# keras-team/keras-rs

Hardware: AMD Instinct MI355X
Metric: embedding lookups/sec + DCN fwd+bwd step time, 26-table DLRM batch 65 536 (higher is better)
Workload: dtype bf16; 1 GPU; C3 DLRM-small: 26 tables x 1000000 rows x 128 (bf16), global batch 65536, multi-hot ml_perf lengths (sum L = 214), uniform ids, DotInteraction(F=27) + 3 x FeatureCross(d=3456, projection=512), fused Adagrad on tables; global_batch=65536, parallelism=single GPU

## Files before the change

### include/krs.h

```cpp
#ifndef KRS_H_
#define KRS_H_

#include <stddef.h>
#include <stdint.h>

#ifdef __cplusplus
extern "C" {
#endif

#define KRS_VERSION 100

typedef enum krs_status {
  KRS_OK = 0,
  KRS_ERR_INVALID = -1,
  KRS_ERR_UNSUPPORTED = -2,
  KRS_ERR_LAUNCH = -3,
  KRS_ERR_WORKSPACE = -4
} krs_status;

typedef enum krs_dtype { KRS_F32 = 0, KRS_BF16 = 1, KRS_I8 = 2 } krs_dtype;
typedef enum krs_itype { KRS_I32 = 0, KRS_I64 = 1 } krs_itype;

typedef enum krs_combiner { KRS_SUM = 0, KRS_MEAN = 1, KRS_SQRTN = 2 } krs_combiner;

// ... 178 lines not shown

enum {
  KRS_GEMM_KERNEL_NONE = 0, KRS_GEMM_KERNEL_GENERIC = 1, KRS_GEMM_KERNEL_MFMA = 2, KRS_GEMM_KERNEL_GLDS = 3,
  KRS_GEMM_KERNEL_TN_GLDS = 4, KRS_GEMM_KERNEL_PP256 = 5, KRS_GEMM_KERNEL_PP256_KSTRIDED = 6, KRS_GEMM_KERNEL_PP64 = 7,
  KRS_GEMM_KERNEL_THIN = 8, KRS_GEMM_KERNEL_ROWDOT = 9, KRS_GEMM_KERNEL_SMALLK = 10
};
enum { KRS_GEMM_REDUCE_NONE = 0, KRS_GEMM_REDUCE_SCALAR = 1, KRS_GEMM_REDUCE_VEC4 = 2, KRS_GEMM_REDUCE_VEC8 = 3 };
typedef struct krs_gemm_route {
  int32_t kernel;
  int32_t splits;
  int32_t reduce;
  int32_t epilogue;
  int32_t ep_vec;
  int32_t thin_width;
  int32_t thin_is_a;
} krs_gemm_route;
int krs_gemm_last_route(krs_gemm_route* route);
int krs_gemm_plan_route(const void* a, int64_t lda, int a_is_km, const void* b, int64_t ldb, int b_is_nk, const void* c,
                        int64_t ldc, int64_t m, int64_t n, int64_t k, int in_dtype, int out_dtype,
                        const krs_gemm_epilogue* epilogue, size_t workspace_bytes, krs_gemm_route* route);

enum { KRS_GEMM_OPT_PIPELINE = 0 };
int krs_gemm_set_option(int key, int value);

enum { KRS_EMBED_OPT_PLAN = 2, KRS_EMBED_OPT_HOTROWS = 3, KRS_EMBED_OPT_RANK = 4, KRS_EMBED_OPT_APPLY_DEPTH = 5 };
int krs_embed_set_option(int key, int value);

size_t krs_colsum_workspace_bytes(int64_t m, int64_t n);
int krs_cross_epilogue_fwd(const void* u, const void* x0, const void* x, void* y,
                           int64_t m, int64_t n, int64_t ld, float diag_scale,
                           int dtype, void* stream);
int krs_cross_epilogue_bwd(const void* g, const void* u, const void* x0, const void* x,
                           void* du, void* dx0, int dx0_accumulate, void* dxd,
                           float* dbias,
                           int64_t m, int64_t n, int64_t ld, float diag_scale, int act,
                           int dtype, void* workspace, size_t workspace_bytes, void* stream);

// ... 215 lines not shown
```

### keras_rs_amd/_lib.py

```python

from __future__ import annotations

import ctypes as C
import os

import numpy as np
import torch

_HERE = os.path.dirname(os.path.abspath(__file__))
LIB_PATH = os.environ.get("KRS_LIB", os.path.join(_HERE, "libkrs_hip.so"))

F32, BF16, I8 = 0, 1, 2
I32, I64 = 0, 1
SUM, MEAN, SQRTN = 0, 1, 2
COMBINERS = {"sum": SUM, "mean": MEAN, "sqrtn": SQRTN}
ACT_NONE, ACT_RELU, ACT_SIGMOID, ACT_TANH = 0, 1, 2, 3
FLAG_ID_OUT_OF_RANGE = 1
FLAG_BAD_OFFSETS = 2
FLAG_CAPACITY_OVERFLOW = 4
FLAG_NONFINITE_ROW = 8
MAX_LIST = 4096

TABLE_DT = np.dtype(
    [("weights", "<u8"), ("slot", "<u8"), ("row_base", "<i8"), ("vocab", "<i4"), ("lr", "<f4")]
# ... 13 lines not shown
        ("act", C.c_int32),
        ("diag_scale", C.c_float),
        ("x0", C.c_void_p),
        ("x", C.c_void_p),
        ("ldx", C.c_int64),
        ("u_out", C.c_void_p),
        ("ldu", C.c_int64),
        ("r", C.c_void_p),
        ("ldr", C.c_int64),
        ("beta", C.c_float),
    ]


class GemmRoute(C.Structure):
    _fields_ = [(name, C.c_int32) for name in
                ("kernel", "splits", "reduce", "epilogue", "ep_vec", "thin_width", "thin_is_a")]


class GemmQ8Route(C.Structure):
    _fields_ = [(name, C.c_int32) for name in ("kernel", "ep_vec", "k_tail", "epilogue")]


class EmbedFwdRoute(C.Structure):
    _fields_ = [(name, C.c_int32) for name in
                ("kernel", "lpr", "has_w", "stream", "hot_rows", "bpg", "table_dtype", "out_dtype")] + [("blocks", C.c_int64)]


class DotRoute(C.Structure):
    _fields_ = [(name, C.c_int32) for name in
                ("kernel", "dtype", "ks", "fr", "self", "multi", "acc", "ng", "lps_log2", "spw", "launches",
                 "lds_bytes")] + [("blocks", C.c_int64)]
# ... 203 lines not shown
```

### keras_rs_amd/csrc/gemm.hip

```cpp
#include <algorithm>
#include <cstdlib>
#include <cstring>

#include "gemm_device.h"
#include "gemm_plan.h"
#include "gemm_ring64.h"

namespace krs {
namespace {

constexpr int BM = gplan::kTile, BN = gplan::kTile;
constexpr int ROW_BYTES = gplan::kRowBytes;
constexpr int TILE_BYTES = gplan::kTileBytes;

template <int ES>
__device__ __forceinline__ void load_kstrided(const char* base, int64_t ld, int64_t row0, int64_t k0,
                                              int64_t rows, int64_t kk, u32x4 (&r)[4]) {
  constexpr int RPB = 16 / ES;
  constexpr int NRB = BM / RPB;
  const int t = threadIdx.x;
  const int rb = t % NRB;
  const int kb = t / NRB;
  const int64_t row = row0 + rb * RPB;
#pragma unroll
// ... 24 lines not shown
      const int j = jj;
      const int w = j >> 1;
      uint32_t lo, hi;
      if (j & 1) {
        lo = (r[0][w] >> 16) | (r[1][w] & 0xffff0000u);
        hi = (r[2][w] >> 16) | (r[3][w] & 0xffff0000u);
      } else {
        lo = (r[0][w] & 0xffffu) | (r[1][w] << 16);
        hi = (r[2][w] & 0xffffu) | (r[3][w] << 16);
      }
      *reinterpret_cast<uint2*>(tile + lds_chunk_off<true>(rb * 8 + j, kb >> 1) + (kb & 1) * 8) = make_uint2(lo, hi);
    }
  }
}

template <int EPI, int NPFC>
__device__ __forceinline__ void gemm_epilogue_wave128_pre(const GemmParams& p, f32x16 (&acc)[2][2][2], float* stage,
                                                          int64_t wm0, int64_t wn0, int split, EpiOperands (&o)[4]) {
  static_assert(NPFC == 2 || NPFC == 4, "two or four chunks of operands are fetched ahead");
  epi_process<EPI>(p, acc[0][0], o[0], stage, wm0, wn0, split);
  if constexpr (NPFC == 2) epi_prefetch<EPI>(p, o[2], wm0 + 64, wn0);
  epi_process<EPI>(p, acc[0][1], o[1], stage, wm0 + 32, wn0, split);
  if constexpr (NPFC == 2) epi_prefetch<EPI>(p, o[3], wm0 + 96, wn0);
  epi_process<EPI>(p, acc[1][0], o[2], stage, wm0 + 64, wn0, split);
  epi_process<EPI>(p, acc[1][1], o[3], stage, wm0 + 96, wn0, split);
}

template <int EPI>
__device__ __forceinline__ void gemm_epilogue(const GemmParams& p, f32x16 (&acc)[2][2], char* smem, int64_t m0,
                                              int64_t n0, int split) {
  const int wave = threadIdx.x >> 6;
  gemm_epilogue_wave<EPI>(p, acc, reinterpret_cast<float*>(smem) + wave * (32 * 68), m0 + (wave >> 1) * 64,
                          n0 + (wave & 1) * 64, split);
}

template <int ES, bool A_KM, bool B_NK, int EPI>
__global__ __launch_bounds__(256, 3) void gemm_mfma_kernel(const GemmParams p) {
  extern __shared__ __attribute__((aligned(16))) char smem[];
  constexpr int BK = ROW_BYTES / ES;
  auto tile_a = [&](int) -> char* { return smem; };
// ... 397 lines not shown
}
template <int N>
__device__ __forceinline__ void pp_lgkm_wait(u32x4 (&fa)[4], u32x4 (&fb)[2]) {
  asm volatile("s_waitcnt lgkmcnt(%6)"
               : "+v"(fa[0]), "+v"(fa[1]), "+v"(fa[2]), "+v"(fa[3]), "+v"(fb[0]), "+v"(fb[1])
               : "n"(N));
}

struct RingMmaBf16 {
  f32x16 (&acc)[2][2][2];
  __device__ __forceinline__ void operator()(int i, int j, const u32x4& fa, const u32x4& fb) const {
    f32x16& d = acc[i >> 1][i & 1][j];
    d = __builtin_amdgcn_mfma_f32_32x32x16_bf16(__builtin_bit_cast(bf16x8, fa), __builtin_bit_cast(bf16x8, fb), d, 0, 0, 0);
  }
};
template <int EPI> constexpr int kRingEpiChunks = EPI == 2 ? 4 : EPI == 1 ? 2 : 0;
template <int EPI> constexpr int kRingEpiLoads = kRingEpiChunks<EPI> * (EPI == 1 ? 8 : 4);

template <bool TN, int NSTG, int EPI>
__global__ __launch_bounds__(512) void gemm_pp256_kernel(const GemmParams p, int mt, int nt) {
  extern __shared__ __attribute__((aligned(16))) char smem[];
  constexpr int TM = 256, TN_ = 256;
  typedef const __attribute__((address_space(1))) void* gptr;
  typedef __attribute__((address_space(3))) void* lptr;

  const int lane = threadIdx.x & 63;
  const int wave = __builtin_amdgcn_readfirstlane(threadIdx.x >> 6);
  const int grp = wave >> 2;
  const int wm = grp, wn = wave & 3;
  const int64_t xcd = blockIdx.x & 7, slot = blockIdx.x >> 3;
  int64_t m0, n0, kbeg = 0, nkb;
// ... 203 lines not shown
  }
  lds_dma_retired<NPF>();
  float* stage_f = reinterpret_cast<float*>(smem) + wave * (32 * 68);
  if constexpr (EPI >= 3) {
    gemm_epilogue_wave128_crossbwd<(EPI == 4 || EPI == 6) ? 1 : (EPI == 7 ? 2 : (EPI >= 8 ? 3 : 0)),
                                   EPI == 3 || EPI == 4 || EPI == 7, EPI < 9, EPI != 9>(
        p, acc, stage_f, m0 + wm * 128, n0 + wn * 64, (m0 >> 8) * 2 + wm);
    return;
  }
  if constexpr (NPFC > 0)
    gemm_epilogue_wave128_pre<EPI, NPFC>(p, acc, stage_f, m0 + wm * 128, n0 + wn * 64, split, opf);
  else
    gemm_epilogue_wave128<EPI>(p, acc, stage_f, m0 + wm * 128, n0 + wn * 64, split);
}

template <int EPI>
__global__ __launch_bounds__(512) void gemm_pp64_kernel(const GemmParams p, int nt) {
  extern __shared__ __attribute__((aligned(16))) char smem[];
  constexpr int TM = 256, TN_ = 256;
  const int lane = threadIdx.x & 63;
  const int wave = __builtin_amdgcn_readfirstlane(threadIdx.x >> 6);
  const int wm = wave >> 2, wn = wave & 3;
  const int64_t xcd = blockIdx.x & 7, slot_id = blockIdx.x >> 3;
  const int64_t tslot = slot_id / p.splits;
  const int split = (int)(slot_id - tslot * p.splits);
  const int64_t m_tile = (tslot / nt) * 8 + xcd;
  if (m_tile * TM >= p.m) return;
  const int64_t m0 = m_tile * TM, n0 = (tslot % nt) * TN_;
  const int64_t kbeg = (int64_t)split * p.k_per_split;
  const int64_t nb = (min(p.k, kbeg + p.k_per_split) - kbeg) / 64;

  f32x16 acc[2][2][2];
#pragma unroll
  for (int h = 0; h < 2; ++h)
#pragma unroll
    for (int i = 0; i < 2; ++i)
#pragma unroll
      for (int j = 0; j < 2; ++j)
#pragma unroll
        for (int r = 0; r < 16; ++r) acc[h][i][j][r] = 0.0f;
  constexpr int NPFC = kRingEpiChunks<EPI>;
  EpiOperands opf[4];
  ring64_main_loop<2, kRingEpiLoads<EPI>>(smem, p, m0, n0, kbeg, nb, lane, wave, RingMmaBf16{acc}, [&]() {
#pragma unroll
    for (int c = 0; c < NPFC; ++c) epi_prefetch<EPI>(p, opf[c], m0 + wm * 128 + c * 32, n0 + wn * 64);
  });
  float* stage_f = reinterpret_cast<float*>(smem) + wave * (32 * 68);
  if constexpr (EPI >= 3) {
    gemm_epilogue_wave128_crossbwd<(EPI == 4 || EPI == 6) ? 1 : (EPI == 7 ? 2 : (EPI >= 8 ? 3 : 0)),
                                   EPI == 3 || EPI == 4 || EPI == 7, EPI < 9, EPI != 9>(
        p, acc, stage_f, m0 + wm * 128, n0 + wn * 64, (m0 >> 8) * 2 + wm);
    return;
  }
  if constexpr (NPFC > 0)
    gemm_epilogue_wave128_pre<EPI, NPFC>(p, acc, stage_f, m0 + wm * 128, n0 + wn * 64, split, opf);
  else
    gemm_epilogue_wave128<EPI>(p, acc, stage_f, m0 + wm * 128, n0 + wn * 64, split);
}

template <int ES, int NT>
__global__ __launch_bounds__(256) void gemm_thin_kernel(const GemmParams p, int thin_is_a) {
  typedef typename std::conditional<ES == 2, uint16_t, float>::type elem_t;
  __shared__ __attribute__((aligned(16))) float thin[128][NT];
  const elem_t* wide_p = reinterpret_cast<const elem_t*>(thin_is_a ? p.b : p.a);
  const elem_t* thin_p = reinterpret_cast<const elem_t*>(thin_is_a ? p.a : p.b);
  const int64_t ldw = thin_is_a ? p.ldb : p.lda, ldt = thin_is_a ? p.lda : p.ldb;
  const int64_t n_wide = thin_is_a ? p.n : p.m;
  const int n_thin = (int)(thin_is_a ? p.m : p.n);
  const int64_t col = (int64_t)blockIdx.x * 256 + threadIdx.x;
  const int64_t ccol = col < n_wide ? col : n_wide - 1;
// ... 188 lines not shown
    const float bv = p.b_nk ? ld_elem(p.b, in_dtype, j * p.ldb + kk) : ld_elem(p.b, in_dtype, kk * p.ldb + j);
    acc = fmaf(av, bv, acc);
  }
  epilogue_store(p, i, j, acc);
}

int g_pipe = -1;
int gemm_pipe() {
  if (g_pipe < 0) {
    const char* e = getenv("KRS_GEMM_PIPE");
    g_pipe = e ? atoi(e) : 4;
    if (g_pipe != 0 && g_pipe != 5) g_pipe = 4;
  }
  return g_pipe;
}

template <int First, int Last, class F>
int with_epilogue(int e, F&& f) {
  if constexpr (First < Last) {
    if (e != First) return with_epilogue<First + 1, Last>(e, f);
  }
  return f(std::integral_constant<int, First>());
}

}
}

using namespace krs;

extern "C" int krs_gemm_set_option(int key, int value) {
  if (key == KRS_GEMM_OPT_PIPELINE) {
    KRS_REQUIRE(value == 0 || value == 4 || value == 5, "krs_gemm_set_option: pipeline must be 0, 4 or 5");
    g_pipe = value;
    return KRS_OK;
  }
  return fail(KRS_ERR_INVALID, "krs_gemm_set_option: unknown key %d", key);
}

extern "C" size_t krs_gemm_workspace_bytes(int64_t m, int64_t n, int64_t k, int a_is_km) {
  return gplan::plan_workspace_bytes(m, n, k, a_is_km != 0);
}

namespace krs {
namespace {
static_assert(gplan::kRingLds == 4 * pp::STAGE && gplan::kRing64Lds == ring64::NSLOT * ring64::SLOT, "the planner's LDS bytes");

thread_local krs_gemm_route g_route = {};

int gemm_plan(const void* a, int64_t lda, int a_is_km, const void* b, int64_t ldb, int b_is_nk, const void* c, int64_t ldc,
              int64_t m, int64_t n, int64_t k, int in_dtype, int out_dtype, const krs_gemm_epilogue* ep,
              size_t workspace_bytes, bool allow_split, gplan::GemmCall& call, gplan::GemmPlan& pl) {
  KRS_REQUIRE(a && b && c, "krs_gemm: null operand");
  KRS_REQUIRE(m >= 0 && n >= 0 && k >= 0, "krs_gemm: negative size");
  KRS_REQUIRE((in_dtype == KRS_F32 || in_dtype == KRS_BF16) && (out_dtype == KRS_F32 || out_dtype == KRS_BF16),
              "krs_gemm: bad dtype");
  if (ep && ep->x0) KRS_REQUIRE(ep->x, "krs_gemm: cross epilogue needs x with x0");
  static const bool tn128 = getenv("KRS_GEMM_TN128") != nullptr;
  call = gplan::GemmCall();
  call.m = m; call.n = n; call.k = k; call.a_km = a_is_km != 0; call.b_nk = b_is_nk != 0;
  call.es = in_dtype == KRS_BF16 ? 2 : 4; call.out_dtype = out_dtype;
  call.lda = lda; call.ldb = ldb; call.ldc = ldc; call.al_a = al16(a); call.al_b = al16(b); call.al_c = al16(c);
  gplan::set_epilogue(call, ep);
  call.workspace_bytes = workspace_bytes; call.allow_split = allow_split; call.pipe = gemm_pipe(); call.tn128 = tn128;
  pl = gplan::plan_gemm(call);
  if (pl.status == KRS_ERR_WORKSPACE)
    return fail(pl.status, "krs_gemm: split-K needs %zu workspace bytes, got %zu", pl.need, workspace_bytes);
  if (pl.status != KRS_OK) return fail(pl.status, "krs_gemm: the shape needs a grid beyond the launch limits");
  return KRS_OK;
}

template <int ES>
int gemm_launch(const GemmParams& p, const gplan::GemmPlan& pl, int in_dtype, hipStream_t st) {
  const krs_gemm_route& rt = pl.route;
  const dim3 grid((unsigned)pl.grid[0], (unsigned)pl.grid[1], (unsigned)pl.grid[2]), block((unsigned)pl.block);
  switch (rt.kernel) {
    case KRS_GEMM_KERNEL_PP64:
      return with_epilogue<0, 2>(rt.epilogue, [&](auto E) {
        return launch_lds<gemm_pp64_kernel<E>>("gemm_pp64_kernel", grid, block, pl.lds, st, p, pl.nt);
      });
    case KRS_GEMM_KERNEL_PP256:
      return with_epilogue<0, 2>(rt.epilogue, [&](auto E) {
        return launch_lds<gemm_pp256_kernel<false, 4, E>>("gemm_pp256_kernel", grid, block, pl.lds, st, p, 0, pl.nt);
      });
    case KRS_GEMM_KERNEL_PP256_KSTRIDED:
      return launch_lds<gemm_pp256_kernel<true, 4, 0>>("gemm_pp256_kernel (K-strided operands)", grid, block, pl.lds, st, p,
                                                       pl.mt, pl.nt);
    case KRS_GEMM_KERNEL_TN_GLDS:
      return launch_lds<gemm_tn_glds_kernel<0>>("gemm_tn_glds_kernel", grid, block, pl.lds, st, p, pl.mt, pl.nt);
    case KRS_GEMM_KERNEL_GLDS:
      return with_epilogue<0, 2>(rt.epilogue, [&](auto E) {
        return launch_lds<gemm_glds_kernel<ES, E>>("gemm_glds_kernel", grid, block, pl.lds, st, p);
      });
    case KRS_GEMM_KERNEL_MFMA:
      return with_epilogue<0, 2>(rt.epilogue, [&](auto E) {
// ... 97 lines not shown
                     gplan::CrossBwdPlan* plan_only = nullptr) {
  const bool store_g = g_out != nullptr;
  if (dense && !g_out) { g_out = dz; ldg = ld; }
  if (!r) { ldr = n; beta = 0.0f; }
  KRS_REQUIRE(dtype == KRS_BF16 || dtype == KRS_F32, "%s: bad dtype", who);
  KRS_REQUIRE(m >= 0 && n >= 0 && k > 0 && ld >= n && ldg >= n && ldr >= n, "%s: bad sizes", who);
  krs_gemm_epilogue ep;
  memset(&ep, 0, sizeof(ep));
  ep.r = r; ep.ldr = ldr; ep.beta = beta;
  gplan::CrossBwdPlan cb;
  if (m > 0 && n > 0) {
    gplan::GemmCall call;
    if (int rc = gemm_plan(a, lda, 0, bt, ldb, 1, g_out, ldg, m, n, k, dtype, dtype, r ? &ep : nullptr, 0, false, call, cb.product))
      return rc;
    gplan::plan_cross_bwd(cb, r != nullptr, ld, al16(x0) && al16(u) && al16(dz) && al16(dx0) && al16(u_upper), dense, store_g,
                          dx0 != nullptr, dx0_accumulate != 0, u_upper != nullptr);
  }
  if (plan_only) { *plan_only = cb; return KRS_OK; }
  if (dbias) KRS_REQUIRE(workspace_bytes >= krs_gemm_cross_bwd_workspace_bytes(m, n) && (workspace || m == 0 || n == 0),
                         "%s: workspace too small (krs_gemm_cross_bwd_workspace_bytes)", who);
  hipStream_t st = reinterpret_cast<hipStream_t>(stream);
  if (m == 0 || n == 0) {
    if (dbias && n > 0) KRS_HIP(hipMemsetAsync(dbias, 0, (size_t)n * sizeof(float), st));
    return KRS_OK;
  }
  if (cb.route == KRS_CROSS_BWD_TWO_CALL) {
    cb_route = cb.route;
    if (int rc = gemm_run(a, lda, 0, bt, ldb, 1, g_out, ldg, m, n, k, dtype, dtype, r ? &ep : nullptr, nullptr, 0, stream,
                          false))
      return rc;
    KRS_REQUIRE(ldg == ld, "%s: the two-call form needs one row stride for G, x0, u, dz and dx0", who);
// ... 4 lines not shown
      if (int rc = krs_cross_epilogue_bwd(r, u_upper, x0, x0, nullptr, dx0, 0, nullptr, nullptr, m, n, ld, 0.0f, KRS_ACT_NONE,
                                          dtype, nullptr, 0, stream)) return rc;
      dx0_accumulate = 1;
    }
    return krs_cross_epilogue_bwd(g_out, u, x0, x0, dz, dx0, dx0_accumulate, fold_direct ? dx0 : nullptr, dbias, m, n,
                                  ld, 0.0f, act, dtype, workspace, workspace_bytes, stream);
  }
  GemmParams p = gemm_params(a, lda, false, bt, ldb, true, g_out, ldg, m, n, k, KRS_BF16, &ep);
  p.ep_vec = 1;
  p.f_x0 = x0; p.f_u = u; p.f_uup = u_upper; p.f_dz = dz; p.f_dx0 = dx0; p.f_ld = ld; p.f_act = act; p.f_fold = fold_direct != 0;
  p.f_partial = dbias ? reinterpret_cast<float*>(workspace) : nullptr;
  const gplan::GemmPlan& pl = cb.product;
  const dim3 grid256((unsigned)pl.grid[0]), block((unsigned)pl.block);
  cb_route = cb.route; cb_epilogue = cb.epilogue;
  const int rc = with_epilogue<3, 10>(cb.epilogue, [&](auto E) {
    return cb.route == KRS_CROSS_BWD_PP64
               ? launch_lds<gemm_pp64_kernel<E>>("gemm_pp64_kernel (fused cross backward)", grid256, block, pl.lds, st, p, pl.nt)
               : launch_lds<gemm_pp256_kernel<false, 4, E>>("gemm_pp256_kernel (fused cross backward)", grid256, block, pl.lds,
                                                            st, p, 0, pl.nt);
  });
  if (rc != KRS_OK) return rc;
  return dbias ? finish_colsum(p.f_partial, 2 * ceil_div(m, 256), n, dbias, st) : KRS_OK;
}

extern "C" int krs_gemm_cross_bwd_plan_route(const void* a, int64_t lda, const void* bt, int64_t ldb, const void* r,
                                             int64_t ldr, float beta, void* g_out, int64_t ldg, const void* x0, const void* u,
                                             void* dz, void* dx0, int64_t ld, int dx0_accumulate, const void* u_upper,
                                             int64_t m, int64_t n, int64_t k, int dtype, int* epilogue) {
  gplan::CrossBwdPlan cb;
  const int rc = cross_bwd("krs_gemm_cross_bwd_plan_route", x0 == nullptr, a, lda, bt, ldb, r, ldr, beta, g_out, ldg, x0, u, dz,
                           dx0, ld, dx0_accumulate, u_upper, 0, nullptr, m, n, k, KRS_ACT_NONE, dtype, nullptr, 0, nullptr, &cb);
  if (epilogue) *epilogue = cb.epilogue;
  return rc ? rc : cb.route;
}
// ... 26 lines not shown
```

### keras_rs_amd/csrc/gemm_device.h

```cpp
#ifndef KRS_GEMM_DEVICE_H_
#define KRS_GEMM_DEVICE_H_

#include "gemm_plan.h"
#include "krs_dense_common.h"

namespace krs {
namespace {

typedef __bf16 bf16x8 __attribute__((ext_vector_type(8)));
typedef float f32x16 __attribute__((ext_vector_type(16)));
typedef uint32_t u32x4 __attribute__((ext_vector_type(4)));

struct GemmParams {
  const char* a; int64_t lda; int a_km;
  const char* b; int64_t ldb; int b_nk;
  char* c; int64_t ldc;
  int64_t m, n, k;
  int out_dtype;
  krs_gemm_epilogue ep;
  int has_ep;
  int splits; int64_t k_per_split; float* slabs;
  int ep_vec;
  const void* f_x0; const void* f_u; const void* f_uup; void* f_dz; void* f_dx0; float* f_partial; int64_t f_ld; int f_act; int f_fold;
};
// ... 120 lines not shown
    }
    if (e.r) {
      float rv[8];
      load8(e.r, odt, i * e.ldr + j, rv);
#pragma unroll
      for (int q = 0; q < 8; ++q) v[q] += e.beta * rv[q];
    }
  }
  store8(p.c, odt, i * p.ldc + j, v);
}


struct EpiOperands {
  uint4 ex[4], ex0[4];
};

template <int EPI>
__device__ __forceinline__ void epi_prefetch(const GemmParams& p, EpiOperands& o, int64_t row0, int64_t wn0) {
  if constexpr (EPI == 1 || EPI == 2) {
    const int lane = threadIdx.x & 63;
    const int64_t gnc = min(wn0 + (lane & 7) * 8, p.n - 8);
#pragma unroll
    for (int it = 0; it < 4; ++it) {
      const int64_t gmc = min(row0 + it * 8 + (lane >> 3), p.m - 1);
      if constexpr (EPI == 1) {
        o.ex[it] = load8_bf16_nt(p.ep.x, gmc * p.ep.ldx + gnc);
        o.ex0[it] = load8_bf16_nt(p.ep.x0, gmc * p.ep.ldx + gnc);
      } else {
        o.ex[it] = load8_bf16_nt(p.ep.r, gmc * p.ep.ldr + gnc);
      }
    }
  }
}

template <int EPI>
__device__ __forceinline__ void epi_process(const GemmParams& p, f32x16 (&acc2)[2], const EpiOperands& o, float* stage,
                                            int64_t row0, int64_t wn0, int split) {
  const int lane = threadIdx.x & 63;
  const int frow = lane & 31;
  const int fhalf = lane >> 5;
  constexpr int SST = 68;
  const int ec = (lane & 7) * 8;
  const int64_t gn = wn0 + ec;
#pragma unroll
  for (int j = 0; j < 2; ++j)
#pragma unroll
    for (int r = 0; r < 16; ++r)
      stage[((r & 3) + 8 * (r >> 2) + 4 * fhalf) * SST + j * 32 + frow] = acc2[j][r];
  __builtin_amdgcn_fence(__ATOMIC_ACQ_REL, "wavefront");
#pragma unroll
  for (int it = 0; it < 4; ++it) {
    const int er = it * 8 + (lane >> 3);
    const int64_t gm = row0 + er;
    if (gm >= p.m || gn >= p.n) continue;
    float v[8];
    const float4 v0 = *reinterpret_cast<const float4*>(stage + er * SST + ec);
    const float4 v1 = *reinterpret_cast<const float4*>(stage + er * SST + ec + 4);
    v[0] = v0.x; v[1] = v0.y; v[2] = v0.z; v[3] = v0.w; v[4] = v1.x; v[5] = v1.y; v[6] = v1.z; v[7] = v1.w;
    if constexpr (EPI == 1) {
      if (p.ep.bias) {
        const float4 b0 = *reinterpret_cast<const float4*>(p.ep.bias + gn);
        const float4 b1 = *reinterpret_cast<const float4*>(p.ep.bias + gn + 4);
        v[0] += b0.x; v[1] += b0.y; v[2] += b0.z; v[3] += b0.w;
        v[4] += b1.x; v[5] += b1.y; v[6] += b1.z; v[7] += b1.w;
      }
      if (p.ep.act != KRS_ACT_NONE) {
#pragma unroll
        for (int q = 0; q < 8; ++q) v[q] = apply_act(p.ep.act, v[q]);
      }
      if (p.ep.u_out) store8_bf16_nt(p.ep.u_out, gm * p.ep.ldu + gn, v);
      float xv[8], x0v[8];
      unpack_bf16x8(o.ex[it], xv);
      unpack_bf16x8(o.ex0[it], x0v);
#pragma unroll
      for (int q = 0; q < 8; ++q) v[q] = x0v[q] * (v[q] + p.ep.diag_scale * xv[q]) + xv[q];
      store8_bf16_nt(p.c, gm * p.ldc + gn, v);
    } else if constexpr (EPI == 2) {
      float rv[8];
      unpack_bf16x8(o.ex[it], rv);
#pragma unroll
      for (int q = 0; q < 8; ++q) v[q] += p.ep.beta * rv[q];
      store8_bf16_nt(p.c, gm * p.ldc + gn, v);
    } else if (p.splits > 1) {
      float* dst = p.slabs + ((int64_t)split * p.m + gm) * p.n + gn;
      if (p.ep_vec) {
        *reinterpret_cast<float4*>(dst) = v0;
        *reinterpret_cast<float4*>(dst + 4) = v1;
      } else {
// ... 65 lines not shown
```

### keras_rs_amd/csrc/gemm_plan.h

```cpp
#ifndef KRS_GEMM_PLAN_H_
#define KRS_GEMM_PLAN_H_

#include <algorithm>
#include <cstddef>
#include <cstdint>

#include "../../include/krs.h"

namespace krs {

inline bool al16(const void* q) { return (reinterpret_cast<uintptr_t>(q) & 15) == 0; }

namespace gplan {

constexpr int kTile = 128, kRowBytes = 128;
constexpr int kLdsStride = kRowBytes + 16, kTileBytes = kTile * kLdsStride;
constexpr int kBigTile = 256, kCUs = 256;
constexpr int kFillTiles = 192;
constexpr int kRingBlock = 32, kRingDepth = 4;
constexpr int kRing64Block = 64, kRing64Depth = 3;
constexpr int kRingMinK = 256;
constexpr int kRingSplitMinK = 2048, kSplitMinK = 512;
constexpr int kGldsMinK = 1024;
constexpr int kThinMax = 16, kThinMinK = 1024, kThinMaxSplits = 128;
constexpr int kWgradMinK = 4096, kMaxSplits = 64;
constexpr int kGeneralMinK = 4096, kGeneralSplitK = 1024, kGeneralWgs = 1024;
constexpr int kRowdotMaxN = 8, kRowdotMinK = 32, kRowdotMinM = 1024, kRowdotRows = 16;
constexpr int kSmallkMaxK = 16, kSmallkMaxN = 1024, kSmallkRows = 64, kSmallkMinMN = 1 << 16;
constexpr size_t kRingLds = 4 * 32768, kRing64Lds = 5 * 32768, kGldsLds = 4 * kTile * kRowBytes;
constexpr int64_t kMaxGridThreads = 0xffffffffll, kMaxGridYZ = 65535;

inline int64_t cdiv(int64_t a, int64_t b) { return (a + b - 1) / b; }
inline int64_t round_up(int64_t a, int64_t b) { return cdiv(a, b) * b; }

struct GemmCall {
  int64_t m = 0, n = 0, k = 0, lda = 0, ldb = 0, ldc = 0, ldx = 0, ldu = 0, ldr = 0;
  bool a_km = false, b_nk = false;
  int es = 2, out_dtype = KRS_BF16, act = KRS_ACT_NONE;
  bool al_a = true, al_b = true, al_c = true, al_bias = true, al_x0 = true, al_x = true, al_u = true, al_r = true;
  bool has_ep = false, bias = false, x0 = false, u_out = false, r = false;
  size_t workspace_bytes = 0;
  bool allow_split = true;
  int pipe = 4;
  bool tn128 = false;
};

inline void set_epilogue(GemmCall& c, const krs_gemm_epilogue* ep) {
  if (!ep) return;
  c.has_ep = true; c.act = ep->act; c.bias = ep->bias != nullptr; c.al_bias = al16(ep->bias);
  c.x0 = ep->x0 != nullptr; c.al_x0 = al16(ep->x0); c.al_x = al16(ep->x); c.ldx = ep->ldx;
  c.u_out = ep->u_out != nullptr; c.al_u = al16(ep->u_out); c.ldu = ep->ldu;
  c.r = ep->r != nullptr; c.al_r = al16(ep->r); c.ldr = ep->ldr;
}

struct GemmPlan {
  krs_gemm_route route = {};
  int status = KRS_OK;
  size_t need = 0, lds = 0;
  int64_t k_per_split = 0, grid[3] = {1, 1, 1}, reduce_grid = 0;
  int block = 256, mt = 0, nt = 0;
};

inline bool thin_shape(int64_t m, int64_t n, int64_t k) { return k >= kThinMinK && std::min(m, n) <= kThinMax; }

inline int pick_splits(int64_t m, int64_t n, int64_t k, bool a_km, bool ring_ok) {
// ... 87 lines not shown
      p.lds = ring ? kRingLds : kGldsLds;
    } else {
      rt.kernel = KRS_GEMM_KERNEL_MFMA;
      p.lds = 2 * kTileBytes;
    }
    if (p.lds == kRingLds || p.lds == kRing64Lds) p.block = 512;
    if (rt.kernel == KRS_GEMM_KERNEL_GLDS || rt.kernel == KRS_GEMM_KERNEL_MFMA) {
      p.grid[0] = (c.a_km ? cdiv(m, kTile) : round_up(cdiv(m, kTile), 8)) * cdiv(n, kTile);
      p.grid[2] = s;
    }
    if (rt.kernel != KRS_GEMM_KERNEL_PP256_KSTRIDED && rt.kernel != KRS_GEMM_KERNEL_TN_GLDS && c.has_ep && rt.ep_vec &&
        s == 1 && c.out_dtype == KRS_BF16 && n >= 8) {
      if (c.x0 && !c.r) rt.epilogue = 1;
      else if (c.r && !c.x0 && !c.bias && c.act == KRS_ACT_NONE) rt.epilogue = 2;
    }
    const bool vec4 = !c.has_ep && c.out_dtype == KRS_F32 && n % 4 == 0 && c.ldc % 4 == 0 && c.al_c;
    if (s > 1) rt.reduce = vec4 ? KRS_GEMM_REDUCE_VEC4 : (rt.ep_vec ? KRS_GEMM_REDUCE_VEC8 : KRS_GEMM_REDUCE_SCALAR);
  } else if (tn && thin_shape(m, n, k)) {
    if (!split(pick_splits(m, n, k, true, false), 1)) p.need = 0;
    const int64_t n_thin = std::min(m, n);
    rt.kernel = KRS_GEMM_KERNEL_THIN;
    rt.thin_is_a = m <= n;
    rt.thin_width = n_thin <= 1 ? 1 : (n_thin <= 4 ? 4 : (n_thin <= 8 ? 8 : 16));
    p.grid[0] = cdiv(std::max(m, n), 256);
    p.grid[1] = rt.splits;
    if (rt.splits > 1) rt.reduce = KRS_GEMM_REDUCE_SCALAR;
  } else if (!c.a_km && n <= kRowdotMaxN && k >= kRowdotMinK && m >= kRowdotMinM) {
    rt.kernel = KRS_GEMM_KERNEL_ROWDOT;
    p.grid[0] = cdiv(m, kRowdotRows);
  } else if (!c.a_km && k <= kSmallkMaxK && n % 8 == 0 && n <= kSmallkMaxN && m * n >= kSmallkMinMN) {
    rt.kernel = KRS_GEMM_KERNEL_SMALLK;
    p.grid[0] = cdiv(m, kSmallkRows);
    p.lds = (size_t)k * n * sizeof(float);
  } else {
    rt.kernel = KRS_GEMM_KERNEL_GENERIC;
    p.grid[0] = cdiv(m * n, 256);
  }
  if (rt.reduce) p.reduce_grid = cdiv(m * (rt.reduce == KRS_GEMM_REDUCE_VEC4 ? n / 4 : rt.reduce == KRS_GEMM_REDUCE_VEC8 ? n / 8 : n), 256);
  if (p.grid[0] * p.block > kMaxGridThreads || p.reduce_grid * 256 > kMaxGridThreads || p.grid[1] > kMaxGridYZ || p.grid[2] > kMaxGridYZ)
    return refuse(KRS_ERR_UNSUPPORTED, 0);
  return p;
}

struct CrossBwdPlan {
  int route = KRS_CROSS_BWD_NONE, epilogue = 0;
  GemmPlan product;
};

inline void plan_cross_bwd(CrossBwdPlan& cb, bool has_r, int64_t ld, bool al_streams, bool dense, bool store_g, bool has_dx0,
                           bool dx0_accumulate, bool has_u_upper) {
  const krs_gemm_route& rt = cb.product.route;
  cb.route = rt.kernel == KRS_GEMM_KERNEL_PP64 ? KRS_CROSS_BWD_PP64 : KRS_CROSS_BWD_PP256;
  cb.epilogue = 0;
  if ((rt.kernel != KRS_GEMM_KERNEL_PP64 && rt.kernel != KRS_GEMM_KERNEL_PP256) || rt.splits != 1 || !rt.ep_vec || ld % 8 != 0 ||
      !al_streams)
    cb.route = rt.kernel == KRS_GEMM_KERNEL_NONE ? KRS_CROSS_BWD_NONE : KRS_CROSS_BWD_TWO_CALL;
  else if (dense) cb.epilogue = store_g ? 10 : 9;
  else if (has_u_upper) cb.epilogue = 7;
  else if (has_r) cb.epilogue = dx0_accumulate ? 4 : 3;
  else cb.epilogue = !has_dx0 ? 8 : (dx0_accumulate ? 6 : 5);
}

}
}
#endif
```

### keras_rs_amd/dense_ops.py

```python

from __future__ import annotations

import ctypes as C
from typing import Sequence

import torch

from keras_rs_amd import _lib as L
from keras_rs_amd import probe

ACTS = {None: L.ACT_NONE, "linear": L.ACT_NONE, "relu": L.ACT_RELU, "sigmoid": L.ACT_SIGMOID,
        "tanh": L.ACT_TANH}


def gemm(a: torch.Tensor, b: torch.Tensor, *, a_is_km: bool = False, b_is_nk: bool = False,
         out_dtype: torch.dtype | None = None, bias: torch.Tensor | None = None, act: int = L.ACT_NONE,
         diag_scale: float = 0.0, x0: torch.Tensor | None = None, x: torch.Tensor | None = None,
         want_u: bool = False, r: torch.Tensor | None = None, beta: float = 1.0,
         out: torch.Tensor | None = None):
    a = L.rowmajor(a, "gemm A")
    b = L.rowmajor(b, "gemm B")
    if a.dtype != b.dtype:
        raise L.KrsError("gemm: A and B must share a dtype")
    m, k = (a.shape[1], a.shape[0]) if a_is_km else (a.shape[0], a.shape[1])
# ... 160 lines not shown
GEMM_REDUCES = {0: None, 1: "scalar", 2: "vec4", 3: "vec8"}


def _route_dict(rt) -> dict:
    return dict(kernel=GEMM_KERNELS[rt.kernel], splits=int(rt.splits), reduce=GEMM_REDUCES[rt.reduce],
                epilogue=int(rt.epilogue), ep_vec=bool(rt.ep_vec), thin_width=int(rt.thin_width),
                thin_is_a=bool(rt.thin_is_a))


def last_gemm_route() -> dict:
    rt = L.GemmRoute()
    L.lib().krs_gemm_last_route(C.byref(rt))
    return _route_dict(rt)


def plan_gemm_route(a, lda, a_is_km, b, ldb, b_is_nk, c, ldc, m, n, k, in_dtype, out_dtype, epilogue=None,
                    workspace_bytes=0):
    rt = L.GemmRoute()
    rc = L.lib().krs_gemm_plan_route(a, lda, int(a_is_km), b, ldb, int(b_is_nk), c, ldc, m, n, k, in_dtype, out_dtype,
                                     C.byref(epilogue) if epilogue is not None else None, int(workspace_bytes), C.byref(rt))
    return int(rc), _route_dict(rt)


GEMM_Q8_KERNELS = {0: None, 1: "generic", 2: "tile128", 3: "ring"}


def _q8_route_dict(rt) -> dict:
    return dict(kernel=GEMM_Q8_KERNELS[rt.kernel], ep_vec=bool(rt.ep_vec), k_tail=bool(rt.k_tail), epilogue=int(rt.epilogue))


# ... 285 lines not shown
```

Measured before the change: 1.498 billion lookups/s.

## Add epilogue schedules for PP64 cross GEMM: LDS landing, x-is-x0, stagger

Adds schedule variants to the PP64 ring GEMM epilogue. Operands for later chunks are landed in LDS through global_load_lds, and bias is hoisted into registers during the main loop. When x aliases x0, a specialised epilogue loads only one operand stream. An optional stagger mode rotates the n-tile order and delays odd slots so epilogue memory traffic does not collide across CUs. The default schedule (1) turns on landing and x_is_x0 for cross-forward GEMMs, which adds template variants and LDS usage and relies on inline asm vmcnt accounting.

```diff
diff --git a/include/krs.h b/include/krs.h
--- a/include/krs.h
+++ b/include/krs.h
@@ -216,13 +216,15 @@
   int32_t ep_vec;
   int32_t thin_width;
   int32_t thin_is_a;
+  int32_t schedule;
 } krs_gemm_route;
+enum { KRS_GEMM_SCHED_LDS_LANDING = 1, KRS_GEMM_SCHED_STAGGER = 2, KRS_GEMM_SCHED_X_IS_X0 = 4 };
 int krs_gemm_last_route(krs_gemm_route* route);
 int krs_gemm_plan_route(const void* a, int64_t lda, int a_is_km, const void* b, int64_t ldb, int b_is_nk, const void* c,
                         int64_t ldc, int64_t m, int64_t n, int64_t k, int in_dtype, int out_dtype,
                         const krs_gemm_epilogue* epilogue, size_t workspace_bytes, krs_gemm_route* route);
 
-enum { KRS_GEMM_OPT_PIPELINE = 0 };
+enum { KRS_GEMM_OPT_PIPELINE = 0, KRS_GEMM_OPT_EPI_SCHEDULE = 1 };
 int krs_gemm_set_option(int key, int value);
 
 enum { KRS_EMBED_OPT_PLAN = 2, KRS_EMBED_OPT_HOTROWS = 3, KRS_EMBED_OPT_RANK = 4, KRS_EMBED_OPT_APPLY_DEPTH = 5 };
diff --git a/keras_rs_amd/_lib.py b/keras_rs_amd/_lib.py
--- a/keras_rs_amd/_lib.py
+++ b/keras_rs_amd/_lib.py
@@ -51,7 +51,11 @@
 
 class GemmRoute(C.Structure):
     _fields_ = [(name, C.c_int32) for name in
-                ("kernel", "splits", "reduce", "epilogue", "ep_vec", "thin_width", "thin_is_a")]
+                ("kernel", "splits", "reduce", "epilogue", "ep_vec", "thin_width", "thin_is_a", "schedule")]
+
+
+GEMM_OPT_PIPELINE, GEMM_OPT_EPI_SCHEDULE = 0, 1
+GEMM_SCHED_LDS_LANDING, GEMM_SCHED_STAGGER, GEMM_SCHED_X_IS_X0 = 1, 2, 4
 
 
 class GemmQ8Route(C.Structure):
diff --git a/keras_rs_amd/csrc/gemm.hip b/keras_rs_amd/csrc/gemm.hip
--- a/keras_rs_amd/csrc/gemm.hip
+++ b/keras_rs_amd/csrc/gemm.hip
@@ -62,16 +62,81 @@
   }
 }
 
-template <int EPI, int NPFC>
+template <bool X0>
+__device__ __forceinline__ void epi_settle(EpiOperands& o) {
+#pragma unroll
+  for (int it = 0; it < 4; ++it) {
+    asm volatile("" : "+v"(o.ex[it].x), "+v"(o.ex[it].y), "+v"(o.ex[it].z), "+v"(o.ex[it].w));
+    if constexpr (X0) asm volatile("" : "+v"(o.ex0[it].x), "+v"(o.ex0[it].y), "+v"(o.ex0[it].z), "+v"(o.ex0[it].w));
+  }
+}
+
+template <int EPI, int NPFC, bool PREBIAS = false>
 __device__ __forceinline__ void gemm_epilogue_wave128_pre(const GemmParams& p, f32x16 (&acc)[2][2][2], float* stage,
-                                                          int64_t wm0, int64_t wn0, int split, EpiOperands (&o)[4]) {
+                                                          int64_t wm0, int64_t wn0, int split, EpiOperands (&o)[4],
+                                                          const float* pre_bias = nullptr) {
   static_assert(NPFC == 2 || NPFC == 4, "two or four chunks of operands are fetched ahead");
-  epi_process<EPI>(p, acc[0][0], o[0], stage, wm0, wn0, split);
+  if constexpr (PREBIAS && NPFC == 4) {
+#pragma unroll
+    for (int c = 0; c < 4; ++c) epi_settle<EPI == 1>(o[c]);
+  }
+  epi_process<EPI, PREBIAS>(p, acc[0][0], o[0], stage, wm0, wn0, split, pre_bias);
   if constexpr (NPFC == 2) epi_prefetch<EPI>(p, o[2], wm0 + 64, wn0);
-  epi_process<EPI>(p, acc[0][1], o[1], stage, wm0 + 32, wn0, split);
+  epi_process<EPI, PREBIAS>(p, acc[0][1], o[1], stage, wm0 + 32, wn0, split, pre_bias);
   if constexpr (NPFC == 2) epi_prefetch<EPI>(p, o[3], wm0 + 96, wn0);
-  epi_process<EPI>(p, acc[1][0], o[2], stage, wm0 + 64, wn0, split);
-  epi_process<EPI>(p, acc[1][1], o[3], stage, wm0 + 96, wn0, split);
+  epi_process<EPI, PREBIAS>(p, acc[1][0], o[2], stage, wm0 + 64, wn0, split, pre_bias);
+  epi_process<EPI, PREBIAS>(p, acc[1][1], o[3], stage, wm0 + 96, wn0, split, pre_bias);
+}
+
+__device__ __forceinline__ void epi_land_issue(const GemmParams& p, uint32_t land, int64_t row0, int64_t wn0) {
+  const int lane = threadIdx.x & 63;
+  const int64_t gnc = min(wn0 + (lane & 7) * 8, p.n - 8);
+  const uint16_t* src[8];
+#pragma unroll
+  for (int it = 0; it < 4; ++it) {
+    const int64_t gmc = min(row0 + it * 8 + (lane >> 3), p.m - 1);
+    src[it] = reinterpret_cast<const uint16_t*>(p.ep.x) + gmc * p.ep.ldx + gnc;
+    src[4 + it] = reinterpret_cast<const uint16_t*>(p.ep.x0) + gmc * p.ep.ldx + gnc;
+  }
+#pragma unroll
+  for (int i = 0; i < 8; ++i) {
+    uint32_t keep;
+    asm volatile("s_mov_b32 %0, m0\n\ts_mov_b32 m0, %2\n\ts_nop 0\n\tglobal_load_lds_dwordx4 %1, off nt\n\ts_mov_b32 m0, %0"
+                 : "=&s"(keep)
+                 : "v"(src[i]), "s"(land + i * 1024)
+                 : "memory");
+  }
+}
+template <int BEHIND>
+__device__ __forceinline__ void epi_land_read(const char* land, EpiOperands& o) {
+  static_assert(BEHIND >= 8 && BEHIND < 64, "vmcnt is a 6-bit counter");
+  asm volatile("s_waitcnt vmcnt(%0)" ::"n"(BEHIND) : "memory");
+  const int lane = threadIdx.x & 63;
+#pragma unroll
+  for (int it = 0; it < 4; ++it) {
+    o.ex[it] = *reinterpret_cast<const uint4*>(land + it * 1024 + lane * 16);
+    o.ex0[it] = *reinterpret_cast<const uint4*>(land + 4096 + it * 1024 + lane * 16);
+  }
+}
+__device__ __forceinline__ void gemm_epilogue_wave128_land(const GemmParams& p, f32x16 (&acc)[2][2][2], float* stage, char* land,
+                                                           int64_t wm0, int64_t wn0, int split, EpiOperands (&o)[4],
+                                                           const float* pre_bias) {
+  const uint32_t land_lds = __builtin_amdgcn_readfirstlane((uint32_t)(uintptr_t)(__attribute__((address_space(3))) char*)land);
+  epi_settle<true>(o[0]);
+  epi_settle<true>(o[1]);
+  epi_land_issue(p, land_lds, wm0 + 64, wn0);
+  epi_process<1, true>(p, acc[0][0], o[0], stage, wm0, wn0, split, pre_bias);
+  epi_prefetch<1>(p, o[0], wm0 + 96, wn0);
+  epi_process<1, true>(p, acc[0][1], o[1], stage, wm0 + 32, wn0, split, pre_bias);
+  if (wm0 + 64 <= p.m && wn0 + 64 <= p.n) {
+    if (p.ep.u_out) epi_land_read<8 + 16>(land, o[1]);
+    else epi_land_read<8 + 8>(land, o[1]);
+  } else {
+    epi_land_read<8>(land, o[1]);
+  }
+  epi_process<1, true>(p, acc[1][0], o[1], stage, wm0 + 64, wn0, split, pre_bias);
+  epi_settle<true>(o[0]);
+  epi_process<1, true>(p, acc[1][1], o[0], stage, wm0 + 96, wn0, split, pre_bias);
 }
 
 template <int EPI>
@@ -499,7 +564,7 @@
     d = __builtin_amdgcn_mfma_f32_32x32x16_bf16(__builtin_bit_cast(bf16x8, fa), __builtin_bit_cast(bf16x8, fb), d, 0, 0, 0);
   }
 };
-template <int EPI> constexpr int kRingEpiChunks = EPI == 2 ? 4 : EPI == 1 ? 2 : 0;
+template <int EPI> constexpr int kRingEpiChunks = EPI == 2 || EPI == kEpiCrossXIsX0 ? 4 : EPI == 1 ? 2 : 0;
 template <int EPI> constexpr int kRingEpiLoads = kRingEpiChunks<EPI> * (EPI == 1 ? 8 : 4);
 
 template <bool TN, int NSTG, int EPI>
@@ -733,10 +798,15 @@
     gemm_epilogue_wave128<EPI>(p, acc, stage_f, m0 + wm * 128, n0 + wn * 64, split);
 }
 
-template <int EPI>
+template <int EPI> constexpr int kRingEpiStreams = EPI == 1 ? 4 : EPI == kEpiCrossXIsX0 ? 3 : EPI == 2 ? 2 : 6;
+template <int EPI, int SCHED>
 __global__ __launch_bounds__(512) void gemm_pp64_kernel(const GemmParams p, int nt) {
   extern __shared__ __attribute__((aligned(16))) char smem[];
   constexpr int TM = 256, TN_ = 256;
+  constexpr bool LAND = (SCHED & KRS_GEMM_SCHED_LDS_LANDING) != 0, STAGGER = (SCHED & KRS_GEMM_SCHED_STAGGER) != 0;
+  static_assert(!LAND || EPI == 1, "only the cross build lands operands in LDS");
+  static_assert(!STAGGER || EPI != 0, "the general build keeps the panel order");
+  static_assert(gplan::kEpiStageBytes + gplan::kEpiLandBytes <= gplan::kRing64Lds, "the landing region lies inside the ring");
   const int lane = threadIdx.x & 63;
   const int wave = __builtin_amdgcn_readfirstlane(threadIdx.x >> 6);
   const int wm = wave >> 2, wn = wave & 3;
@@ -745,9 +815,15 @@
   const int split = (int)(slot_id - tslot * p.splits);
   const int64_t m_tile = (tslot / nt) * 8 + xcd;
   if (m_tile * TM >= p.m) return;
-  const int64_t m0 = m_tile * TM, n0 = (tslot % nt) * TN_;
+  const int64_t m0 = m_tile * TM, n0 = (STAGGER ? gplan::ring_tile_of_slot(tslot, nt, true).n_tile : tslot % nt) * TN_;
   const int64_t kbeg = (int64_t)split * p.k_per_split;
   const int64_t nb = (min(p.k, kbeg + p.k_per_split) - kbeg) / 64;
+  if constexpr (STAGGER) {
+    if (blockIdx.x < gplan::kCUs && (slot_id & 1)) {
+      const uint64_t half_period = (uint64_t)nb * 78 + kRingEpiStreams<EPI> * 260, t0 = wall_clock64();
+      for (int i = 0; i < 256 && wall_clock64() - t0 < half_period; ++i) __builtin_amdgcn_s_sleep(16);
+    }
+  }
 
   f32x16 acc[2][2][2];
 #pragma unroll
@@ -760,19 +836,25 @@
         for (int r = 0; r < 16; ++r) acc[h][i][j][r] = 0.0f;
   constexpr int NPFC = kRingEpiChunks<EPI>;
   EpiOperands opf[4];
-  ring64_main_loop<2, kRingEpiLoads<EPI>>(smem, p, m0, n0, kbeg, nb, lane, wave, RingMmaBf16{acc}, [&]() {
+  constexpr bool PREBIAS = LAND || EPI == kEpiCrossXIsX0;
+  float pre_bias[8];
+  ring64_main_loop<2, kRingEpiLoads<EPI> + (PREBIAS ? 2 : 0)>(smem, p, m0, n0, kbeg, nb, lane, wave, RingMmaBf16{acc}, [&]() {
+    if constexpr (PREBIAS) epi_load_bias(p, n0 + wn * 64, pre_bias);
 #pragma unroll
     for (int c = 0; c < NPFC; ++c) epi_prefetch<EPI>(p, opf[c], m0 + wm * 128 + c * 32, n0 + wn * 64);
   });
   float* stage_f = reinterpret_cast<float*>(smem) + wave * (32 * 68);
-  if constexpr (EPI >= 3) {
+  if constexpr (EPI >= 3 && EPI <= 10) {
     gemm_epilogue_wave128_crossbwd<(EPI == 4 || EPI == 6) ? 1 : (EPI == 7 ? 2 : (EPI >= 8 ? 3 : 0)),
                                    EPI == 3 || EPI == 4 || EPI == 7, EPI < 9, EPI != 9>(
         p, acc, stage_f, m0 + wm * 128, n0 + wn * 64, (m0 >> 8) * 2 + wm);
     return;
   }
-  if constexpr (NPFC > 0)
-    gemm_epilogue_wave128_pre<EPI, NPFC>(p, acc, stage_f, m0 + wm * 128, n0 + wn * 64, split, opf);
+  if constexpr (LAND)
+    gemm_epilogue_wave128_land(p, acc, stage_f, smem + gplan::kEpiStageBytes + wave * gplan::kEpiLandWaveBytes, m0 + wm * 128,
+                               n0 + wn * 64, split, opf, pre_bias);
+  else if constexpr (NPFC > 0)
+    gemm_epilogue_wave128_pre<EPI, NPFC, PREBIAS>(p, acc, stage_f, m0 + wm * 128, n0 + wn * 64, split, opf, pre_bias);
   else
     gemm_epilogue_wave128<EPI>(p, acc, stage_f, m0 + wm * 128, n0 + wn * 64, split);
 }
@@ -991,6 +1073,16 @@
   }
   return g_pipe;
 }
+constexpr int kEpiSchedDefault = 1;
+int g_epi_sched = -1;
+int gemm_epi_sched() {
+  if (g_epi_sched < 0) {
+    const char* e = getenv("KRS_GEMM_EPI_SCHEDULE");
+    g_epi_sched = e ? atoi(e) : kEpiSchedDefault;
+    if (g_epi_sched < 0 || g_epi_sched > 3) g_epi_sched = kEpiSchedDefault;
+  }
+  return g_epi_sched;
+}
 
 template <int First, int Last, class F>
 int with_epilogue(int e, F&& f) {
@@ -1009,6 +1101,11 @@
   if (key == KRS_GEMM_OPT_PIPELINE) {
     KRS_REQUIRE(value == 0 || value == 4 || value == 5, "krs_gemm_set_option: pipeline must be 0, 4 or 5");
     g_pipe = value;
+    return KRS_OK;
+  }
+  if (key == KRS_GEMM_OPT_EPI_SCHEDULE) {
+    KRS_REQUIRE(value >= -1 && value <= 3, "krs_gemm_set_option: epilogue schedule must be 0, 1, 2, 3 or -1 (the default)");
+    g_epi_sched = value;
     return KRS_OK;
   }
   return fail(KRS_ERR_INVALID, "krs_gemm_set_option: unknown key %d", key);
@@ -1039,6 +1136,7 @@
   call.lda = lda; call.ldb = ldb; call.ldc = ldc; call.al_a = al16(a); call.al_b = al16(b); call.al_c = al16(c);
   gplan::set_epilogue(call, ep);
   call.workspace_bytes = workspace_bytes; call.allow_split = allow_split; call.pipe = gemm_pipe(); call.tn128 = tn128;
+  call.epi_sched = gemm_epi_sched();
   pl = gplan::plan_gemm(call);
   if (pl.status == KRS_ERR_WORKSPACE)
     return fail(pl.status, "krs_gemm: split-K needs %zu workspace bytes, got %zu", pl.need, workspace_bytes);
@@ -1051,10 +1149,26 @@
   const krs_gemm_route& rt = pl.route;
   const dim3 grid((unsigned)pl.grid[0], (unsigned)pl.grid[1], (unsigned)pl.grid[2]), block((unsigned)pl.block);
   switch (rt.kernel) {
-    case KRS_GEMM_KERNEL_PP64:
-      return with_epilogue<0, 2>(rt.epilogue, [&](auto E) {
-        return launch_lds<gemm_pp64_kernel<E>>("gemm_pp64_kernel", grid, block, pl.lds, st, p, pl.nt);
-      });
+    case KRS_GEMM_KERNEL_PP64: {
+      constexpr int LAND = KRS_GEMM_SCHED_LDS_LANDING, STAG = KRS_GEMM_SCHED_STAGGER, X0 = kEpiCrossXIsX0;
+      const bool stag = (rt.schedule & STAG) != 0;
+      auto run = [&](auto E, auto S) {
+        return launch_lds<gemm_pp64_kernel<E, S>>("gemm_pp64_kernel", grid, block, pl.lds, st, p, pl.nt);
+      };
+      using std::integral_constant;
+      if (rt.epilogue == 0) return run(integral_constant<int, 0>(), integral_constant<int, 0>());
+      if (rt.epilogue == 2)
+        return stag ? run(integral_constant<int, 2>(), integral_constant<int, STAG>())
+                    : run(integral_constant<int, 2>(), integral_constant<int, 0>());
+      if (rt.schedule & KRS_GEMM_SCHED_X_IS_X0)
+        return stag ? run(integral_constant<int, X0>(), integral_constant<int, STAG>())
+                    : run(integral_constant<int, X0>(), integral_constant<int, 0>());
+      if (rt.schedule & LAND)
+        return stag ? run(integral_constant<int, 1>(), integral_constant<int, LAND | STAG>())
+                    : run(integral_constant<int, 1>(), integral_constant<int, LAND>());
+      return stag ? run(integral_constant<int, 1>(), integral_constant<int, STAG>())
+                  : run(integral_constant<int, 1>(), integral_constant<int, 0>());
+    }
     case KRS_GEMM_KERNEL_PP256:
       return with_epilogue<0, 2>(rt.epilogue, [&](auto E) {
         return launch_lds<gemm_pp256_kernel<false, 4, E>>("gemm_pp256_kernel", grid, block, pl.lds, st, p, 0, pl.nt);
@@ -1182,7 +1296,7 @@
     if (int rc = gemm_plan(a, lda, 0, bt, ldb, 1, g_out, ldg, m, n, k, dtype, dtype, r ? &ep : nullptr, 0, false, call, cb.product))
       return rc;
     gplan::plan_cross_bwd(cb, r != nullptr, ld, al16(x0) && al16(u) && al16(dz) && al16(dx0) && al16(u_upper), dense, store_g,
-                          dx0 != nullptr, dx0_accumulate != 0, u_upper != nullptr);
+                          dx0 != nullptr, dx0_accumulate != 0, u_upper != nullptr, gemm_epi_sched());
   }
   if (plan_only) { *plan_only = cb; return KRS_OK; }
   if (dbias) KRS_REQUIRE(workspace_bytes >= krs_gemm_cross_bwd_workspace_bytes(m, n) && (workspace || m == 0 || n == 0),
@@ -1217,10 +1331,13 @@
   const dim3 grid256((unsigned)pl.grid[0]), block((unsigned)pl.block);
   cb_route = cb.route; cb_epilogue = cb.epilogue;
   const int rc = with_epilogue<3, 10>(cb.epilogue, [&](auto E) {
-    return cb.route == KRS_CROSS_BWD_PP64
-               ? launch_lds<gemm_pp64_kernel<E>>("gemm_pp64_kernel (fused cross backward)", grid256, block, pl.lds, st, p, pl.nt)
-               : launch_lds<gemm_pp256_kernel<false, 4, E>>("gemm_pp256_kernel (fused cross backward)", grid256, block, pl.lds,
-                                                            st, p, 0, pl.nt);
+    if (cb.route == KRS_CROSS_BWD_PP64)
+      return cb.stagger ? launch_lds<gemm_pp64_kernel<E, KRS_GEMM_SCHED_STAGGER>>("gemm_pp64_kernel (fused cross backward)",
+                                                                                  grid256, block, pl.lds, st, p, pl.nt)
+                        : launch_lds<gemm_pp64_kernel<E, 0>>("gemm_pp64_kernel (fused cross backward)", grid256, block, pl.lds,
+                                                             st, p, pl.nt);
+    return launch_lds<gemm_pp256_kernel<false, 4, E>>("gemm_pp256_kernel (fused cross backward)", grid256, block, pl.lds, st,
+                                                      p, 0, pl.nt);
   });
   if (rc != KRS_OK) return rc;
   return dbias ? finish_colsum(p.f_partial, 2 * ceil_div(m, 256), n, dbias, st) : KRS_OK;
diff --git a/keras_rs_amd/csrc/gemm_device.h b/keras_rs_amd/csrc/gemm_device.h
--- a/keras_rs_amd/csrc/gemm_device.h
+++ b/keras_rs_amd/csrc/gemm_device.h
@@ -158,16 +158,19 @@
 struct EpiOperands {
   uint4 ex[4], ex0[4];
 };
+constexpr int kEpiCrossXIsX0 = 11;
 
 template <int EPI>
 __device__ __forceinline__ void epi_prefetch(const GemmParams& p, EpiOperands& o, int64_t row0, int64_t wn0) {
-  if constexpr (EPI == 1 || EPI == 2) {
+  if constexpr (EPI == 1 || EPI == 2 || EPI == kEpiCrossXIsX0) {
     const int lane = threadIdx.x & 63;
     const int64_t gnc = min(wn0 + (lane & 7) * 8, p.n - 8);
 #pragma unroll
     for (int it = 0; it < 4; ++it) {
       const int64_t gmc = min(row0 + it * 8 + (lane >> 3), p.m - 1);
-      if constexpr (EPI == 1) {
+      if constexpr (EPI == kEpiCrossXIsX0) {
+        o.ex[it] = load8_bf16_nt(p.ep.x, gmc * p.ep.ldx + gnc);
+      } else if constexpr (EPI == 1) {
         o.ex[it] = load8_bf16_nt(p.ep.x, gmc * p.ep.ldx + gnc);
         o.ex0[it] = load8_bf16_nt(p.ep.x0, gmc * p.ep.ldx + gnc);
       } else {
@@ -177,9 +180,16 @@
   }
 }
 
-template <int EPI>
+__device__ __forceinline__ void epi_load_bias(const GemmParams& p, int64_t wn0, float (&b)[8]) {
+  const float* src = p.ep.bias ? p.ep.bias + min(wn0 + (threadIdx.x & 7) * 8, p.n - 8) : reinterpret_cast<const float*>(p.b);
+  const float4 b0 = *reinterpret_cast<const float4*>(src);
+  const float4 b1 = *reinterpret_cast<const float4*>(src + 4);
+  b[0] = b0.x; b[1] = b0.y; b[2] = b0.z; b[3] = b0.w; b[4] = b1.x; b[5] = b1.y; b[6] = b1.z; b[7] = b1.w;
+}
+
+template <int EPI, bool PREBIAS = false>
 __device__ __forceinline__ void epi_process(const GemmParams& p, f32x16 (&acc2)[2], const EpiOperands& o, float* stage,
-                                            int64_t row0, int64_t wn0, int split) {
+                                            int64_t row0, int64_t wn0, int split, const float* pre_bias = nullptr) {
   const int lane = threadIdx.x & 63;
   const int frow = lane & 31;
   const int fhalf = lane >> 5;
@@ -201,12 +211,17 @@
     const float4 v0 = *reinterpret_cast<const float4*>(stage + er * SST + ec);
     const float4 v1 = *reinterpret_cast<const float4*>(stage + er * SST + ec + 4);
     v[0] = v0.x; v[1] = v0.y; v[2] = v0.z; v[3] = v0.w; v[4] = v1.x; v[5] = v1.y; v[6] = v1.z; v[7] = v1.w;
-    if constexpr (EPI == 1) {
+    if constexpr (EPI == 1 || EPI == kEpiCrossXIsX0) {
       if (p.ep.bias) {
-        const float4 b0 = *reinterpret_cast<const float4*>(p.ep.bias + gn);
-        const float4 b1 = *reinterpret_cast<const float4*>(p.ep.bias + gn + 4);
-        v[0] += b0.x; v[1] += b0.y; v[2] += b0.z; v[3] += b0.w;
-        v[4] += b1.x; v[5] += b1.y; v[6] += b1.z; v[7] += b1.w;
+        if constexpr (PREBIAS) {
+#pragma unroll
+          for (int q = 0; q < 8; ++q) v[q] += pre_bias[q];
+        } else {
+          const float4 b0 = *reinterpret_cast<const float4*>(p.ep.bias + gn);
+          const float4 b1 = *reinterpret_cast<const float4*>(p.ep.bias + gn + 4);
+          v[0] += b0.x; v[1] += b0.y; v[2] += b0.z; v[3] += b0.w;
+          v[4] += b1.x; v[5] += b1.y; v[6] += b1.z; v[7] += b1.w;
+        }
       }
       if (p.ep.act != KRS_ACT_NONE) {
 #pragma unroll
@@ -215,7 +230,7 @@
       if (p.ep.u_out) store8_bf16_nt(p.ep.u_out, gm * p.ep.ldu + gn, v);
       float xv[8], x0v[8];
       unpack_bf16x8(o.ex[it], xv);
-      unpack_bf16x8(o.ex0[it], x0v);
+      unpack_bf16x8(EPI == 1 ? o.ex0[it] : o.ex[it], x0v);
 #pragma unroll
       for (int q = 0; q < 8; ++q) v[q] = x0v[q] * (v[q] + p.ep.diag_scale * xv[q]) + xv[q];
       store8_bf16_nt(p.c, gm * p.ldc + gn, v);
diff --git a/keras_rs_amd/csrc/gemm_plan.h b/keras_rs_amd/csrc/gemm_plan.h
--- a/keras_rs_amd/csrc/gemm_plan.h
+++ b/keras_rs_amd/csrc/gemm_plan.h
@@ -29,6 +29,16 @@
 constexpr int kSmallkMaxK = 16, kSmallkMaxN = 1024, kSmallkRows = 64, kSmallkMinMN = 1 << 16;
 constexpr size_t kRingLds = 4 * 32768, kRing64Lds = 5 * 32768, kGldsLds = 4 * kTile * kRowBytes;
 constexpr int64_t kMaxGridThreads = 0xffffffffll, kMaxGridYZ = 65535;
+constexpr size_t kEpiStageBytes = 8 * 32 * 68 * sizeof(float), kEpiLandWaveBytes = 2 * 32 * 128;
+constexpr size_t kEpiLandBytes = 8 * kEpiLandWaveBytes;
+
+struct RingTile { int64_t panel; int n_tile; };
+constexpr RingTile ring_tile_of_slot(int64_t tslot, int nt, bool stagger) {
+  const int64_t g = tslot / nt;
+  int j = (int)(tslot - g * nt);
+  if (stagger && (g & 1)) j = j + nt / 2 >= nt ? j + nt / 2 - nt : j + nt / 2;
+  return RingTile{g, j};
+}
 
 inline int64_t cdiv(int64_t a, int64_t b) { return (a + b - 1) / b; }
 inline int64_t round_up(int64_t a, int64_t b) { return cdiv(a, b) * b; }
@@ -43,12 +53,15 @@
   bool allow_split = true;
   int pipe = 4;
   bool tn128 = false;
+  bool x_is_x0 = false;
+  int epi_sched = 0;
 };
 
 inline void set_epilogue(GemmCall& c, const krs_gemm_epilogue* ep) {
   if (!ep) return;
   c.has_ep = true; c.act = ep->act; c.bias = ep->bias != nullptr; c.al_bias = al16(ep->bias);
   c.x0 = ep->x0 != nullptr; c.al_x0 = al16(ep->x0); c.al_x = al16(ep->x); c.ldx = ep->ldx;
+  c.x_is_x0 = c.x0 && ep->x == ep->x0;
   c.u_out = ep->u_out != nullptr; c.al_u = al16(ep->u_out); c.ldu = ep->ldu;
   c.r = ep->r != nullptr; c.al_r = al16(ep->r); c.ldr = ep->ldr;
 }
@@ -166,6 +179,10 @@
       if (c.x0 && !c.r) rt.epilogue = 1;
       else if (c.r && !c.x0 && !c.bias && c.act == KRS_ACT_NONE) rt.epilogue = 2;
     }
+    if (rt.kernel == KRS_GEMM_KERNEL_PP64 && rt.epilogue != 0) {
+      if ((c.epi_sched & 1) && rt.epilogue == 1) rt.schedule |= c.x_is_x0 ? KRS_GEMM_SCHED_X_IS_X0 : KRS_GEMM_SCHED_LDS_LANDING;
+      if (c.epi_sched & 2) rt.schedule |= KRS_GEMM_SCHED_STAGGER;
+    }
     const bool vec4 = !c.has_ep && c.out_dtype == KRS_F32 && n % 4 == 0 && c.ldc % 4 == 0 && c.al_c;
     if (s > 1) rt.reduce = vec4 ? KRS_GEMM_REDUCE_VEC4 : (rt.ep_vec ? KRS_GEMM_REDUCE_VEC8 : KRS_GEMM_REDUCE_SCALAR);
   } else if (tn && thin_shape(m, n, k)) {
@@ -196,11 +213,12 @@
 
 struct CrossBwdPlan {
   int route = KRS_CROSS_BWD_NONE, epilogue = 0;
+  bool stagger = false;
   GemmPlan product;
 };
 
 inline void plan_cross_bwd(CrossBwdPlan& cb, bool has_r, int64_t ld, bool al_streams, bool dense, bool store_g, bool has_dx0,
-                           bool dx0_accumulate, bool has_u_upper) {
+                           bool dx0_accumulate, bool has_u_upper, int epi_sched = 0) {
   const krs_gemm_route& rt = cb.product.route;
   cb.route = rt.kernel == KRS_GEMM_KERNEL_PP64 ? KRS_CROSS_BWD_PP64 : KRS_CROSS_BWD_PP256;
   cb.epilogue = 0;
@@ -211,6 +229,7 @@
   else if (has_u_upper) cb.epilogue = 7;
   else if (has_r) cb.epilogue = dx0_accumulate ? 4 : 3;
   else cb.epilogue = !has_dx0 ? 8 : (dx0_accumulate ? 6 : 5);
+  cb.stagger = cb.route == KRS_CROSS_BWD_PP64 && (epi_sched & 2);
 }
 
 }
diff --git a/keras_rs_amd/dense_ops.py b/keras_rs_amd/dense_ops.py
--- a/keras_rs_amd/dense_ops.py
+++ b/keras_rs_amd/dense_ops.py
@@ -198,6 +198,25 @@
     return _route_dict(rt)
 
 
+def _schedule_set(rt) -> frozenset:
+    names = ((L.GEMM_SCHED_LDS_LANDING, "lds_landing"), (L.GEMM_SCHED_STAGGER, "stagger"), (L.GEMM_SCHED_X_IS_X0, "x_is_x0"))
+    return frozenset(name for bit, name in names if rt.schedule & bit)
+
+
+def last_gemm_schedule() -> frozenset:
+    rt = L.GemmRoute()
+    L.lib().krs_gemm_last_route(C.byref(rt))
+    return _schedule_set(rt)
+
+
+def plan_gemm_schedule(a, lda, a_is_km, b, ldb, b_is_nk, c, ldc, m, n, k, in_dtype, out_dtype, epilogue=None,
+                       workspace_bytes=0) -> frozenset:
+    rt = L.GemmRoute()
+    L.lib().krs_gemm_plan_route(a, lda, int(a_is_km), b, ldb, int(b_is_nk), c, ldc, m, n, k, in_dtype, out_dtype,
+                                C.byref(epilogue) if epilogue is not None else None, int(workspace_bytes), C.byref(rt))
+    return _schedule_set(rt)
+
+
 def plan_gemm_route(a, lda, a_is_km, b, ldb, b_is_nk, c, ldc, m, n, k, in_dtype, out_dtype, epilogue=None,
                     workspace_bytes=0):
     rt = L.GemmRoute()
```

Result: faster. 1.518 billion lookups/s (median of 6 runs) (+1.3%).
